# EXLYSHA/Recommendar-Systems

Hardware: AMD Instinct MI355X
Metric: BPR interactions/sec + full-sort items/sec, LightGCN d=64 at 1/2/4/8 MI355X (higher is better)
Workload: dtype f32; 1 GPU; C2: LightGCN K=3 d=64, sports-shaped (35,598 users x 18,357 items per rank), B=2048 per rank, device sampler, fused step; model=LightGCN, n_layers=3, embedding_size=64, global_batch=2048, per_rank_batch=2048, parallelism=single

## Files before the change

### recommendar-systems_amd/csrc/fullsort.hip

```cpp
#include <algorithm>
#include <climits>
#include <cstdlib>

#include "rsx_common.hpp"

namespace rsx {

typedef float floatx16 __attribute__((ext_vector_type(16)));
typedef unsigned long long u64;

constexpr int kCap = 256;
constexpr int kNK = kCap / 64;
constexpr int kSlack = 16;
constexpr int kWarm = 8;
constexpr int kMaxK = 96;

__device__ __forceinline__ unsigned ord_f32(float f) {
    const unsigned u = __float_as_uint(f);
    return (u & 0x80000000u) ? ~u : (u | 0x80000000u);
}
__device__ __forceinline__ float unord_f32(unsigned o) {
    const unsigned u = (o & 0x80000000u) ? (o & 0x7fffffffu) : ~o;
    return __uint_as_float(u);
}
// ... 12 lines not shown
    const unsigned lo = __shfl((unsigned)(v & 0xffffffffu), src, kWave);
    const unsigned hi = __shfl((unsigned)(v >> 32), src, kWave);
    return ((u64)hi << 32) | lo;
}

__device__ __forceinline__ void bitonic128_desc(u64& e0, u64& e1, int lane) {
#pragma unroll
    for (int size = 2; size <= 128; size <<= 1) {
#pragma unroll
        for (int stride = size >> 1; stride > 0; stride >>= 1) {
            if (stride == 64) {
                const u64 mx = e0 > e1 ? e0 : e1;
                const u64 mn = e0 > e1 ? e1 : e0;
                e0 = mx;
                e1 = mn;
            } else {
                const bool lower = (lane & stride) == 0;
                {
                    const u64 pv = shfl_xor_u64(e0, stride);
                    const bool desc = ((lane & size) == 0);
                    const bool keep_max = (lower == desc);
                    e0 = keep_max ? (e0 > pv ? e0 : pv) : (e0 > pv ? pv : e0);
                }
                {
                    const u64 pv = shfl_xor_u64(e1, stride);
                    const bool desc = (((lane + 64) & size) == 0);
                    const bool keep_max = (lower == desc);
                    e1 = keep_max ? (e1 > pv ? e1 : pv) : (e1 > pv ? pv : e1);
                }
            }
        }
    }
}

struct FsArgs {
    const float* U;
    const int64_t* users;
    int64_t nb;
    const float* I;
    int64_t ni;
    const int64_t* mrp;
    const int32_t* mcol;
    int k;
    int n_chunks;
    int64_t chunk_items;
    u64* cand;
    int* ccount;
    float* out_val;
    int64_t* out_idx;
    const __bf16* Ib;
    int n_lists;
    int seg_slots;
    int64_t seg_waves;
    unsigned* lbound;
    uint16_t* samp;
    uint16_t* mcnt1;
};


__device__ __forceinline__ int popc64(u64 x) { return __popcll(x); }
__device__ __forceinline__ u64 lanemask_lt(int lane) { return lane ? (~0ull >> (64 - lane)) : 0ull; }

__device__ __forceinline__ u64 ld_u64_l2(const u64* p) {
    return __hip_atomic_load(p, __ATOMIC_RELAXED, __HIP_MEMORY_SCOPE_AGENT);
}


__device__ __forceinline__ float compact_slot(u64* buf, int n, int k, int lane, int* new_cnt, unsigned lo,
                                              unsigned hi, int slack = -1) {
    asm volatile("s_waitcnt vmcnt(0)" ::: "memory");
    u64 x[kNK];
    unsigned hw[kNK];
#pragma unroll
    for (int q = 0; q < kNK; ++q) {
        x[q] = lane + 64 * q < n ? ld_u64_l2(buf + lane + 64 * q) : 0ull;
        hw[q] = (unsigned)(x[q] >> 32);
    }
    const unsigned diff = lo ^ hi;
    const int top = diff ? 31 - __builtin_clz(diff) : -1;
    unsigned th = top >= 31 ? 0u : (hi >> (top + 1)) << (top + 1);
    for (int bit = top; bit >= 0; --bit) {
        const unsigned c = th | (1u << bit);
        int m = 0;
#pragma unroll
        for (int q = 0; q < kNK; ++q) m += popc64(__ballot(hw[q] >= c));
        if (m >= k) {
            th = c;
            if (m <= k + slack) {
                const u64 lt = lanemask_lt(lane);
                int base = 0;
#pragma unroll
                for (int q = 0; q < kNK; ++q) {
                    const bool kp = x[q] != 0ull && hw[q] >= th;
                    const u64 bq = __ballot(kp);
                    if (kp) buf[base + popc64(bq & lt)] = x[q];
                    base += popc64(bq);
                }
                *new_cnt = base;
                return unord_f32(th);
            }
        }
    }
    int gt = 0, eq = 0;
#pragma unroll
    for (int q = 0; q < kNK; ++q) {
        gt += popc64(__ballot(hw[q] > th));
// ... 237 lines not shown
                    t2[r] = fmaxf(t2[r], lo);
                }
            }
            unsigned th = 0;
            for (int bit = 31; bit >= 0; --bit) {
                const unsigned c = th | (1u << bit);
                int n = 0;
#pragma unroll
                for (int r = 0; r < 16; ++r) n += (int)(ord_f32(t1[r]) >= c) + (int)(ord_f32(t2[r]) >= c);
                n += __shfl_xor(n, 32, kWave);
                if (n >= a.k) th = c;
            }
            if (uvalid && th > 0) {
                const float tb = unord_f32(th - 1);
                tau = tb == 0.f ? -__FLT_DENORM_MIN__ : tb;
            }
            mp = mp0;
            next_mask = nm0;
            load_chunk<D, CW>(ra, a.I, i0 + j, i1, a.ni, h * HALF, i0 + 32 <= i1);
        }
    }

    if (ntiles > 0) {
        floatx16 prev, cur;
        mfma_tile(IntC<0>{}, 0, prev);
        unsigned mb = mask_bits(i0);
        for (int t = 1; t < ntiles; ++t) {
            mfma_tile(IntC<0>{}, t, cur);
            filter(prev, mb, i0 + (int64_t)(t - 1) * 32);
            compact();
            mb = mask_bits(i0 + (int64_t)t * 32);
            prev = cur;
        }
        filter(prev, mb, i0 + (int64_t)(ntiles - 1) * 32);
        compact();
    }
    if (a.n_chunks > 2) {
        u64 need = __ballot(h == 0 && cnt > a.k);
        while (need) {
            const int jj = __ffsll((long long)need) - 1;
            need &= need - 1;
            const int n = __builtin_amdgcn_readlane(cnt, jj);
            const unsigned lo = (unsigned)__builtin_amdgcn_readlane((int)ord_f32(tau), jj);
            const unsigned hi = max((unsigned)__builtin_amdgcn_readlane((int)omax, jj),
                                    (unsigned)__builtin_amdgcn_readlane((int)omax, jj + 32));
            int kept;
            compact_slot(base + (int64_t)jj * rowstep, n, a.k, lane, &kept, lo, hi);
            if (j == jj) cnt = kept;
        }
    }
    if (uvalid && h == 0) a.ccount[bslot * a.n_chunks + chunk] = cnt;
}

constexpr int kScreenWpe = 2;
constexpr int kScreenTop = 3;
template <int D>
constexpr int kAbuf = D <= 64 ? 2 : 1;
typedef __bf16 bf16x8 __attribute__((ext_vector_type(8)));
typedef __bf16 bf16x2 __attribute__((ext_vector_type(2)));
typedef unsigned u32x4 __attribute__((ext_vector_type(4)));
constexpr float kScreenEps = 0.0080f;

template <int D>
constexpr int kScreenRow = D + 16;
constexpr int kScreenPadTiles = 2;

__device__ __forceinline__ unsigned pack_bf16x2(float lo, float hi) {
    const bf16x2 v = {(__bf16)lo, (__bf16)hi};
    return __builtin_bit_cast(unsigned, v);
}
__device__ __forceinline__ bf16x8 pack_bf16x8(float4 p, float4 q) {
    const u32x4 w = {pack_bf16x2(p.x, p.y), pack_bf16x2(p.z, p.w), pack_bf16x2(q.x, q.y), pack_bf16x2(q.z, q.w)};
    return __builtin_bit_cast(bf16x8, w);
}
__device__ __forceinline__ float vmax(float a, float b) {
    float r;
    asm("v_max_f32 %0, %1, %2" : "=v"(r) : "v"(a), "v"(b));
    return r;
}
__device__ __forceinline__ float vmed3(float a, float b, float c) {
    float r;
    asm("v_med3_f32 %0, %1, %2, %3" : "=v"(r) : "v"(a), "v"(b), "v"(c));
    return r;
}

__device__ __forceinline__ unsigned bf16_up(float x) { return (__float_as_uint(x) + 0xffffu) >> 16; }

template <int D>
__global__ __launch_bounds__(256) void fs_prep(const float* __restrict__ I, int64_t ni, int64_t ni_pad,
                                               __bf16* __restrict__ Ib) {
    constexpr int G = D / 4;
    constexpr int DP = kScreenRow<D>;
    const int64_t t = (int64_t)blockIdx.x * 256 + threadIdx.x;
    const int64_t row = t / G;
    const int c = (int)(t % G);
    const float4 v = row < ni ? ld4(I + row * D + 4 * c) : f4(0.f);
    float ss = v.x * v.x + v.y * v.y + v.z * v.z + v.w * v.w;
#pragma unroll
    for (int o = G / 2; o > 0; o >>= 1) ss += __shfl_xor(ss, o, kWave);
    if (row >= ni_pad) return;
    __bf16* r = Ib + row * DP;
    *reinterpret_cast<uint2*>(r + 4 * c) = make_uint2(pack_bf16x2(v.x, v.y), pack_bf16x2(v.z, v.w));
    if (c == 0) {
        const u32x4 z = {0u, 0u, 0u, 0u};
        u32x4 w = z;
        w[0] = bf16_up(sqrtf(ss) * 1.0001f);
        *reinterpret_cast<u32x4*>(r + D) = w;
        *reinterpret_cast<u32x4*>(r + D + 8) = z;
    }
}

template <int D, int ND>
__device__ __forceinline__ void exact_dots(const float* const (&u)[ND], const float* const (&v)[ND], float (&out)[ND]) {
    float acc[ND];
#pragma unroll
    for (int n = 0; n < ND; ++n) acc[n] = 0.f;
#pragma unroll 4
    for (int c = 0; c < D; c += 4) {
        float4 x[ND], y[ND];
#pragma unroll
        for (int n = 0; n < ND; ++n) {
            x[n] = *reinterpret_cast<const float4*>(u[n] + c);
            y[n] = ld4(v[n] + c);
        }
#pragma unroll
        for (int n = 0; n < ND; ++n) {
            acc[n] = fmaf(x[n].x, y[n].x, acc[n]);
            acc[n] = fmaf(x[n].y, y[n].y, acc[n]);
            acc[n] = fmaf(x[n].z, y[n].z, acc[n]);
            acc[n] = fmaf(x[n].w, y[n].w, acc[n]);
        }
    }
#pragma unroll
    for (int n = 0; n < ND; ++n) out[n] = acc[n];
}

constexpr int kDrainPer = 1;
constexpr int kQueueCap = 64 * kDrainPer + 1024;
constexpr int kMaskCap = 32;
constexpr int kMaskStride = kMaskCap + 1;

template <int D, int PH>
__device__ __forceinline__ void screen_segment(const FsArgs& a, int64_t ub, int chunk, int li, int ta, int tz,
                                               float* urows, unsigned* queue, int* lcnt, unsigned* lomax,
                                               int* mlds) {
    constexpr int HALF = D / 2;
    constexpr int NM = D / 16;
    constexpr int DP = kScreenRow<D>;
    constexpr int US = D + 4;
    const int lane = threadIdx.x, j = lane & 31, h = lane >> 5;
    const int64_t ublock = ub * 32;
    const int64_t bslot = ublock + j;
    const bool uvalid = bslot < a.nb;
    const int64_t urow = uvalid ? (a.users ? a.users[bslot] : bslot) : 0;
    const int64_t c0 = (int64_t)chunk * a.chunk_items;
    const int64_t i0 = c0 + (int64_t)ta * 32;
    const int64_t i1 = min(min(a.ni, c0 + a.chunk_items), c0 + (int64_t)tz * 32);
    const int ntiles = tz - ta;
    u64* const base = a.cand + (ublock * a.n_lists + li) * (int64_t)kCap;
    const int64_t rowstep = (int64_t)a.n_lists * kCap;

    u32x4 bu[NM + 1];
    float ss = 0.f;
    float* const myrow = urows + j * US;
#pragma unroll
    for (int s = 0; s < NM; ++s) {
        const float4 p = uvalid ? ld4(a.U + urow * D + h * HALF + 8 * s) : f4(0.f);
        const float4 q = uvalid ? ld4(a.U + urow * D + h * HALF + 8 * s + 4) : f4(0.f);
        ss += p.x * p.x + p.y * p.y + p.z * p.z + p.w * p.w + q.x * q.x + q.y * q.y + q.z * q.z + q.w * q.w;
        bu[s] = u32x4{pack_bf16x2(p.x, p.y), pack_bf16x2(p.z, p.w), pack_bf16x2(q.x, q.y), pack_bf16x2(q.z, q.w)};
        if constexpr (PH == 2) {
            *reinterpret_cast<float4*>(myrow + h * HALF + 8 * s) = p;
            *reinterpret_cast<float4*>(myrow + h * HALF + 8 * s + 4) = q;
        }
    }
    ss += __shfl_xor(ss, 32, kWave);
    const unsigned cmb = bf16_up(kScreenEps * sqrtf(ss) * 1.0001f);
    bu[NM] = u32x4{h == 0 ? (cmb | 0x8000u) : 0u, 0u, 0u, 0u};
    __syncthreads();

    int64_t mp = 0, me = 0, mq = 0;
    if (uvalid && a.mrp) {
        int64_t lo = a.mrp[urow], hi = a.mrp[urow + 1];
        me = hi;
        auto first_ge = [&](int64_t l, int64_t r, int64_t x) __attribute__((always_inline)) {
            while (l < r) {
                const int64_t mid = (l + r) >> 1;
                if ((int64_t)a.mcol[mid] < x) l = mid + 1; else r = mid;
            }
            return l;
        };
        mp = first_ge(lo, hi, i0);
        mq = first_ge(mp, hi, i1);
    }
    const int64_t mcount = mq - mp;
    const int kk = a.k + (int)mcount;
    const bool mfree = __ballot(uvalid && kk > 32 * kScreenTop) == 0ull;
    const bool mlds_ok = __ballot(mcount > kMaskCap) == 0ull;
    int* const ml = mlds + j * kMaskStride;
    if (mlds_ok) {
        int v[kMaskCap / 2];
        if (mcount > 0) {
#pragma unroll
            for (int q = 0; q < kMaskCap / 2; ++q) v[q] = a.mcol[mp + min((int64_t)(2 * q + h), mcount - 1)];
        }
#pragma unroll
        for (int q = 0; q < kMaskCap / 2; ++q) ml[2 * q + h] = 2 * q + h < mcount ? v[q] : INT_MAX;
        if (h == 0) ml[kMaskCap] = INT_MAX;
    }
    const int64_t mp0 = mp;
    int next_mask = INT_MAX, after = INT_MAX, mcur = 0;
    auto mask_start = [&]() __attribute__((always_inline)) {
        const int nm = mlds_ok ? ml[0] : (mp0 < me ? a.mcol[mp0] : INT_MAX);
        const int af = (!mlds_ok && mp0 + 1 < me) ? a.mcol[mp0 + 1] : INT_MAX;
        mcur = 0;
        mp = mp0;
        next_mask = nm;
        after = af;
    };
    __syncthreads();
    mask_start();
    auto mask_bits = [&](auto form, int64_t tb) __attribute__((always_inline)) -> unsigned {
        constexpr int M = decltype(form)::value;
        unsigned mb = 0;
        if constexpr (M == 1) {
            while ((int64_t)next_mask < tb + 32) {
                mb |= 1u << (unsigned)((int64_t)next_mask - tb);
                next_mask = ml[++mcur];
            }
        } else if constexpr (M == 2) {
            while ((int64_t)next_mask < tb + 32) {
                mb |= 1u << (unsigned)((int64_t)next_mask - tb);
                ++mp;
                next_mask = after;
                after = mp + 1 < me ? a.mcol[mp + 1] : INT_MAX;
            }
        }
        return mb;
    };
    constexpr int NB = kAbuf<D>;
    static_assert(NB == 1 || NB == 2, "the ring below is written for one or two buffers");
    u32x4 ra[NB][NM + 1];
    const __bf16* const a0 = a.Ib + (i0 + j) * DP;
    const __bf16* anext = a0;
    auto load_a = [&](auto par) __attribute__((always_inline)) {
        constexpr int P = decltype(par)::value % NB;
        const u32x4* p = reinterpret_cast<const u32x4*>(anext + h * HALF);
#pragma unroll
        for (int s = 0; s < NM; ++s) ra[P][s] = p[s];
        ra[P][NM] = *reinterpret_cast<const u32x4*>(anext + D + 8 * h);
        anext += 32 * DP;
    };
    auto tile = [&](auto par, int t, floatx16& acc) __attribute__((always_inline)) {
        constexpr int P = decltype(par)::value % NB;
        if constexpr (NB > 1) load_a(IntC<(P + NB - 1) % NB>{});
#pragma unroll
        for (int r = 0; r < 16; ++r) acc[r] = 0.f;
#pragma unroll
        for (int s = 0; s <= NM; ++s)
            acc = __builtin_amdgcn_mfma_f32_32x32x16_bf16(__builtin_bit_cast(bf16x8, ra[P][s]),
                                                          __builtin_bit_cast(bf16x8, bu[s]), acc, 0, 0, 0);
        if constexpr (NB == 1) load_a(IntC<0>{});
    };
    auto prime = [&]() __attribute__((always_inline)) {
        anext = a0;
        if (ntiles <= 0) return;
        load_a(IntC<0>{});
    };
    auto sweep = [&](auto&& body) __attribute__((always_inline)) {
        for (int t = 0; t < ntiles; t += NB) {
            body(IntC<0>{}, t);
            if constexpr (NB > 1)
                if (t + 1 < ntiles) body(IntC<1>{}, t + 1);
        }
    };

    float t1[16], t2[16], t3[16];
#pragma unroll
    for (int r = 0; r < 16; ++r) t1[r] = t2[r] = t3[r] = -INFINITY;
    auto p1_issue = [&](auto form, auto par, int t, floatx16& acc) __attribute__((always_inline)) -> unsigned {
        const unsigned mb = mask_bits(form, i0 + (int64_t)t * 32);
        tile(par, t, acc);
        return mb;
    };
    auto p1_update = [&](auto form, int t, floatx16& acc, unsigned mb) __attribute__((always_inline)) {
        const int64_t tb = i0 + (int64_t)t * 32;
        const int rem = (int)(i1 - tb);
        if (rem < 32 || (decltype(form)::value != 0 && __ballot(mb != 0u) != 0ull)) {
            const unsigned mbh = mb >> (4 * h);
            const int remh = rem - 4 * h;
#pragma unroll
            for (int r = 0; r < 16; ++r) {
                const int io = (r & 3) + 8 * (r >> 2);
                acc[r] = io >= remh ? -INFINITY : (((mbh >> io) & 1u) ? -1e10f : acc[r]);
            }
        }
#pragma unroll
        for (int r = 0; r < 16; ++r) {
            t3[r] = vmed3(t2[r], t3[r], acc[r]);
            t2[r] = vmed3(t1[r], t2[r], acc[r]);
            t1[r] = vmax(t1[r], acc[r]);
        }
    };
    auto pass1 = [&](auto form, auto par, int t) __attribute__((always_inline)) {
        floatx16 acc;
        const unsigned mb = p1_issue(form, par, t, acc);
        p1_update(form, t, acc, mb);
    };
    auto sweep1 = [&](auto form) __attribute__((always_inline)) {
        sweep([&](auto par, int t) __attribute__((always_inline)) { pass1(form, par, t); });
    };
    if constexpr (PH == 1) {
        prime();
        if (mfree) sweep1(IntC<0>{});
        else if (mlds_ok) sweep1(IntC<1>{});
        else sweep1(IntC<2>{});
        if (uvalid) {
            auto s16 = [](float x) __attribute__((always_inline)) -> unsigned {
                return x == -INFINITY ? 0u : ord_f32(x) >> 16;
            };
            uint4* dst = reinterpret_cast<uint4*>(a.samp + ((bslot * a.n_lists + li) * 96 + h * 48));
#pragma unroll
            for (int q = 0; q < 6; ++q) {
                unsigned w[4];
#pragma unroll
                for (int e = 0; e < 4; ++e) {
                    const int v0 = 8 * q + 2 * e, v1 = v0 + 1;
                    const float x0 = v0 < 16 ? t1[v0] : v0 < 32 ? t2[v0 - 16] : t3[v0 - 32];
                    const float x1 = v1 < 16 ? t1[v1] : v1 < 32 ? t2[v1 - 16] : t3[v1 - 32];
                    w[e] = s16(x0) | (s16(x1) << 16);
                }
                dst[q] = make_uint4(w[0], w[1], w[2], w[3]);
            }
            if (h == 0) a.mcnt1[bslot * a.n_lists + li] = (uint16_t)(mfree ? min(mcount, (int64_t)0xfffe) : 0);
        }
        return;
    }
    const unsigned th = uvalid ? a.lbound[bslot] : 0u;
    float tau = -INFINITY;
    if (th > ord_f32(-INFINITY)) {
        const float tb = unord_f32(th - 1);
        tau = tb == 0.f ? -__FLT_DENORM_MIN__ : tb;
    }

    bu[NM] = u32x4{h == 0 ? cmb : 0u, 0u, 0u, 0u};
    mask_start();
    int cnt = 0;
    unsigned omax = 0;
    if (lane < 32) {
        lcnt[lane] = 0;
        lomax[lane] = 0u;
    }
    int qn = 0;
    auto compact = [&]() __attribute__((always_inline)) {
        u64 need = __ballot(h == 0 && cnt > kCap - 64 * kDrainPer);
        while (need) {
            const int jj = __ffsll((long long)need) - 1;
            need &= need - 1;
            const int nn = __builtin_amdgcn_readlane(cnt, jj);
            const unsigned lo = (unsigned)__builtin_amdgcn_readlane((int)ord_f32(tau), jj);
            const unsigned hi = (unsigned)__builtin_amdgcn_readlane((int)omax, jj);
            int kept;
            const float nt = compact_slot(base + (int64_t)jj * rowstep, nn, a.k, lane, &kept, lo, hi, kSlack);
            if (j == jj) {
                tau = nt;
                cnt = kept;
            }
            if (lane == jj) lcnt[jj] = kept;
        }
    };
    const u64 ltm = lanemask_lt(lane);
    auto drain = [&](bool all) __attribute__((always_inline)) {
        constexpr int G = 64 * kDrainPer;
        int g = 0;
        while (qn - g >= G || (all && qn > g)) {
            const int n = min(G, qn - g);
            __syncthreads();
            unsigned e[kDrainPer];
            int ju[kDrainPer];
            float tj[kDrainPer], sc[kDrainPer];
            const float* up[kDrainPer];
            const float* vp[kDrainPer];
#pragma unroll
            for (int q = 0; q < kDrainPer; ++q) {
                e[q] = lane + 64 * q < n ? queue[g + lane + 64 * q] : 0u;
                ju[q] = (int)(e[q] & 31u);
                tj[q] = __shfl(tau, ju[q], kWave);
                up[q] = urows + ju[q] * US;
                vp[q] = a.I + (int64_t)(e[q] >> 6) * D;
            }
            if (lane < n) {
                exact_dots<D, kDrainPer>(up, vp, sc);
            }
#pragma unroll
            for (int q = 0; q < kDrainPer; ++q) {
                const float v = (e[q] & 32u) ? -1e10f : sc[q];
                if (lane + 64 * q < n && v > tj[q]) {
                    const int pos = atomicAdd(&lcnt[ju[q]], 1);
                    const u64 key = make_key(v, (int)(e[q] >> 6));
                    atomicMax(&lomax[ju[q]], (unsigned)(key >> 32));
                    base[(int64_t)ju[q] * rowstep + pos] = key;
                }
            }
            __syncthreads();
            cnt = lcnt[j];
            omax = lomax[j];
            compact();
            g += n;
        }
        const int rest = qn - g;
        if (g > 0 && rest > 0) {
            unsigned v[kDrainPer];
            __syncthreads();
#pragma unroll
            for (int q = 0; q < kDrainPer; ++q) v[q] = lane + 64 * q < rest ? queue[g + lane + 64 * q] : 0u;
            __syncthreads();
#pragma unroll
            for (int q = 0; q < kDrainPer; ++q)
                if (lane + 64 * q < rest) queue[lane + 64 * q] = v[q];
        }
        qn = rest;
    };
    auto pass2 = [&](auto form, auto par, int t) __attribute__((always_inline)) {
        const int64_t tb = i0 + (int64_t)t * 32;
        const unsigned mb = mask_bits(form, tb);
        floatx16 acc;
        tile(par, t, acc);
        const int rem = (int)(i1 - tb);
        const unsigned ebase = ((unsigned)(tb + 4 * h) << 6) | (unsigned)j;
        auto push = [&](bool c, unsigned e) __attribute__((always_inline)) {
            const u64 bal = __ballot(c);
            if (bal) {
                const int rk = __builtin_amdgcn_mbcnt_hi((unsigned)(bal >> 32), __builtin_amdgcn_mbcnt_lo((unsigned)bal, 0u));
                if (c) queue[qn + rk] = e;
                qn += popc64(bal);
            }
        };
        const float tv = uvalid ? tau : INFINITY;
        const unsigned mbh = mb >> (4 * h);
        if (rem < 32 || __ballot(tv < -1e10f) != 0ull) {
            const int remh = rem - 4 * h;
#pragma unroll
            for (int r = 0; r < 16; ++r) {
                const int io = (r & 3) + 8 * (r >> 2);
                acc[r] = io >= remh ? -INFINITY : (((mbh >> io) & 1u) ? -1e10f : acc[r]);
            }
        }
#pragma unroll
        for (int r = 0; r < 16; ++r) {
            const int io = (r & 3) + 8 * (r >> 2);
            push(acc[r] > tv, (ebase + ((unsigned)io << 6)) | (((mbh >> io) & 1u) << 5));
        }
        if (qn >= 64 * kDrainPer) drain(false);
    };
    prime();
    if (mlds_ok) sweep([&](auto par, int t) __attribute__((always_inline)) { pass2(IntC<1>{}, par, t); });
    else sweep([&](auto par, int t) __attribute__((always_inline)) { pass2(IntC<2>{}, par, t); });
    drain(true);
    __syncthreads();
    cnt = lcnt[j];
    omax = lomax[j];
    if (a.n_lists > 8) {
        u64 need = __ballot(h == 0 && cnt > a.k);
        while (need) {
            const int jj = __ffsll((long long)need) - 1;
            need &= need - 1;
            const int nn = __builtin_amdgcn_readlane(cnt, jj);
            const unsigned lo = (unsigned)__builtin_amdgcn_readlane((int)ord_f32(tau), jj);
            const unsigned hi = max((unsigned)__builtin_amdgcn_readlane((int)omax, jj),
                                    (unsigned)__builtin_amdgcn_readlane((int)omax, jj + 32));
            int kept;
            compact_slot(base + (int64_t)jj * rowstep, nn, a.k, lane, &kept, lo, hi);
            if (j == jj) cnt = kept;
        }
    }
    if (uvalid && h == 0) a.ccount[bslot * a.n_lists + li] = cnt;
    __syncthreads();
}

template <int D, int PH>
__global__ __launch_bounds__(64) __attribute__((amdgpu_waves_per_eu(D <= 64 ? kScreenWpe : 1))) void fs_screen(FsArgs a) {
    constexpr int US = D + 4;
    __shared__ __attribute__((aligned(16))) float urows[PH == 1 ? 4 : 32 * US];
    __shared__ unsigned queue[PH == 1 ? 1 : kQueueCap];
    __shared__ int lcnt[32];
    __shared__ unsigned lomax[32];
    __shared__ int mlds[32 * kMaskStride];
    const int64_t n_ub = (a.nb + 31) / 32;
    const int64_t nper = a.seg_waves ? a.seg_waves : n_ub;
    int64_t w;
    int chunk;
    if ((8 % a.n_chunks) == 0) {
        const int64_t b = blockIdx.x, xcd = b & 7, slot = b >> 3;
        chunk = (int)(xcd % a.n_chunks);
        w = slot * (8 / a.n_chunks) + xcd / a.n_chunks;
    } else {
        chunk = (int)(blockIdx.x % a.n_chunks);
        w = blockIdx.x / a.n_chunks;
    }
    if (w >= nper) return;
    const int64_t c0 = (int64_t)chunk * a.chunk_items;
    const int nt = (int)((min(a.ni, c0 + a.chunk_items) - c0 + 31) / 32);
    const int64_t T = n_ub * nt;
    const int64_t lo = a.seg_waves ? w * T / nper : w * nt, hi = a.seg_waves ? (w + 1) * T / nper : (w + 1) * nt;
    const int S = a.seg_slots;
    for (int64_t x = lo; x < hi;) {
        const int64_t ub = x / nt;
        const int t0 = (int)(x - ub * nt);
        const int t1 = (int)min((int64_t)nt, t0 + (hi - x));
        const int64_t wf = ((ub * nt + 1) * nper + T - 1) / T - 1;
        const int seg = a.seg_waves ? (int)(w - wf) : 0;
        screen_segment<D, PH>(a, ub, chunk, chunk * S + seg, t0, t1, urows, queue, lcnt, lomax, mlds);
        if (PH == 2 && t1 == nt) {
            const int j = threadIdx.x & 31;
            const int64_t bslot = ub * 32 + j;
            if (threadIdx.x < 32 && bslot < a.nb)
                for (int q = seg + 1; q < S; ++q) a.ccount[bslot * a.n_lists + chunk * S + q] = 0;
        }
        x += t1 - t0;
    }
}

template <int NW>
__global__ __launch_bounds__(256) void fs_thresh(const uint16_t* __restrict__ samp, const uint16_t* __restrict__ mcnt,
                                                 int nl, int64_t nb, int k, unsigned* __restrict__ lbound) {
    const int lane = threadIdx.x & 63;
    const int64_t b = (int64_t)blockIdx.x * 4 + (threadIdx.x >> 6);
    if (b >= nb) return;
    const unsigned m = lane < nl ? (unsigned)mcnt[b * nl + lane] : 0xffffu;
    const u64 valid = __ballot(m != 0xffffu);
    int mm = m != 0xffffu ? (int)m : 0;
#pragma unroll
    for (int o = 32; o > 0; o >>= 1) mm += __shfl_xor(mm, o, kWave);
    const int kk = k + mm;
    const int nwords = nl * 48;
    const unsigned* __restrict__ w32 = reinterpret_cast<const unsigned*>(samp) + b * nwords;
    unsigned v[2 * NW];
#pragma unroll
    for (int q = 0; q < NW; ++q) {
        const int e = lane + 64 * q;
        const unsigned x = e < nwords ? w32[e] : 0u;
        const bool ok = e < nwords && ((valid >> (e / 48)) & 1ull);
        v[2 * q] = ok ? (x & 0xffffu) : 0u;
        v[2 * q + 1] = ok ? (x >> 16) : 0u;
    }
    unsigned th = 0;
    for (int bit = 15; bit >= 0; --bit) {
        const unsigned c = th | (1u << bit);
        int n = 0;
#pragma unroll
        for (int q = 0; q < 2 * NW; ++q) n += popc64(__ballot(v[q] >= c));
        if (n >= kk) th = c;
    }
    if (lane == 0) lbound[b] = th << 16;
}

template <int E>
__device__ __forceinline__ u64 kth_largest_n(const u64 (&e)[E], int k) {
    unsigned hi = 0u, lo = 0xffffffffu;
#pragma unroll
    for (int m = 0; m < E; ++m) {
        const unsigned w = (unsigned)(e[m] >> 32);
        if (e[m] != 0ull) {
            hi = max(hi, w);
            lo = min(lo, w);
        }
    }
#pragma unroll
    for (int o = kWave / 2; o > 0; o >>= 1) {
// ... 129 lines not shown
            base += popc64(bal);
        }
    } else {
        for (int p0 = 0; p0 < total; p0 += 64) {
            const u64 x = p0 + lane < total ? Ls.at(p0 + lane) : 0ull;
            const bool kp = x != 0ull && x >= T;
            const u64 bal = __ballot(kp);
            if (kp) top[wv][base + popc64(bal & lt)] = x;
            base += popc64(bal);
        }
    }
    __builtin_amdgcn_wave_barrier();
    __builtin_amdgcn_fence(__ATOMIC_SEQ_CST, "wavefront");
    const int kept = base;
    for (int q = lane; q < kept; q += 64) {
        const u64 mine = top[wv][q];
        int r = 0;
        for (int t = 0; t < kept; ++t) r += top[wv][t] > mine;
        a.out_val[b * k + r] = key_score(mine);
        a.out_idx[b * k + r] = (int64_t)key_index(mine);
    }
    for (int q = kept + lane; q < k; q += 64) {
        a.out_val[b * k + q] = -INFINITY;
        a.out_idx[b * k + q] = -1;
    }
}

static void fs_plan(int64_t nb, int64_t ni, int d, int* n_chunks, int64_t* chunk_items) {
    const int64_t waves = (nb + 31) / 32;
    const int64_t target = d <= 64 ? 1900 : 950;
    int64_t s = (target + waves - 1) / waves;
    if (s < 1) s = 1;
    if (s > 16) s = 16;
    int64_t per = (ni + s - 1) / s;
    per = (per + 31) / 32 * 32;
    if (per < 32) per = 32;
    *chunk_items = per;
    *n_chunks = (int)((ni + per - 1) / per);
}

static bool fs_use_screen(int k, int d, int64_t ni) {
    return k <= 64 && (d == 32 || d == 64 || d == 128 || d == 256) && ni < (1ll << 26);
}

static size_t fs_align(size_t x) { return (x + 255) / 256 * 256; }

struct FsLayout {
    int n_chunks;
    int64_t chunk_items;
    bool screen;
    int n_lists, seg_slots;
    int64_t seg_waves;
    int64_t blocks;
};

static int fs_cus() {
    static int n = 0;
    if (!n) {
        int dev = 0, v = 0;
        n = (hipGetDevice(&dev) == hipSuccess &&
             hipDeviceGetAttribute(&v, hipDeviceAttributeMultiprocessorCount, dev) == hipSuccess && v > 0)
                ? v
                : 256;
        (void)hipGetLastError();
    }
    return n;
}

static void screen_plan(int64_t nb, int64_t ni, int wps, int* n_chunks, int64_t* chunk_items) {
    const int64_t n_ub = (nb + 31) / 32;
    const int64_t slots = (int64_t)fs_cus() * 4 * wps;
    int64_t c = slots / n_ub;
    if (c < 1 || n_ub * c * 5 < slots * 4) c = (slots + n_ub - 1) / n_ub;
    if (c < 1) c = 1;
    if (c > 16) c = 16;
    int64_t per = (ni + c - 1) / c;
    per = (per + 31) / 32 * 32;
    *chunk_items = per;
    *n_chunks = (int)((ni + per - 1) / per);
}

static int fs_wps(int d) { return d <= 128 ? 2 : 1; }

static FsLayout fs_layout(int64_t nb, int64_t ni, int k, int d) {
    FsLayout L{};
    const int wps = fs_wps(d);
    L.screen = fs_use_screen(k, d, ni);
    if (L.screen) screen_plan(nb, ni, wps, &L.n_chunks, &L.chunk_items);
    else fs_plan(nb, ni, d, &L.n_chunks, &L.chunk_items);
    L.n_lists = L.n_chunks;
    L.seg_slots = 1;
    const int64_t n_ub = (nb + 31) / 32;
    const int C = L.n_chunks;
    L.blocks = n_ub * C;
    if (L.screen && (8 % C) == 0) {
        const int64_t slots = (int64_t)fs_cus() * 4 * wps;
        const int64_t wc = slots / C;
        if (n_ub * C > slots && wc >= 1) {
            int S = 1;
            bool ok = true;
            for (int c = 0; c < C; ++c) {
                const int64_t nt = (std::min(ni, (int64_t)(c + 1) * L.chunk_items) - (int64_t)c * L.chunk_items + 31) / 32;
                const int64_t m = n_ub * nt / wc;
                if (m < 1) ok = false;
                else S = (int)std::max<int64_t>(S, (nt + m - 1) / m + 1);
            }
            if (ok && C * S <= 8) {
                L.seg_waves = wc;
                L.seg_slots = S;
                L.n_lists = C * S;
                L.blocks = wc * C;
            }
        }
    }
    if ((8 % C) == 0) L.blocks = (L.blocks + 7) / 8 * 8;
    return L;
}

size_t fs_ws(int64_t nb, int64_t ni, int k, int d) {
    const FsLayout L = fs_layout(nb, ni, k, d);
    const int nl = L.n_lists;
    size_t bytes = fs_align((size_t)nb * nl * kCap * sizeof(u64) + (size_t)nb * nl * sizeof(int) + 512);
    if (L.screen) {
        const size_t ni_pad = (size_t)(ni + 31) / 32 * 32;
        bytes += fs_align((ni_pad + 32 * kScreenPadTiles) * (d + 16) * sizeof(__bf16));
        bytes += fs_align((size_t)nb * sizeof(unsigned));
        bytes += fs_align((size_t)nb * L.n_lists * 96 * sizeof(uint16_t));
        bytes += fs_align((size_t)nb * L.n_lists * sizeof(uint16_t));
    }
    return bytes;
}

template <int D>
static int launch_fs(const FsArgs& a, const FsLayout& L, hipStream_t s) {
    const dim3 grid((unsigned)L.blocks);
    if (a.Ib) {
        const int64_t ni_pad = (a.ni + 31) / 32 * 32;
        const int64_t nthr = ni_pad * (D / 4);
        hipLaunchKernelGGL((fs_prep<D>), dim3((unsigned)((nthr + 255) / 256)), dim3(256), 0, s, a.I, a.ni, ni_pad,
                           const_cast<__bf16*>(a.Ib));
        (void)hipMemsetAsync(a.mcnt1, 0xff, (size_t)a.nb * L.n_lists * sizeof(uint16_t), s);
        hipLaunchKernelGGL((fs_screen<D, 1>), grid, dim3(64), 0, s, a);
        {
            const dim3 tg((unsigned)((a.nb + 3) / 4));
            const uint16_t* sp = a.samp;
            const uint16_t* mc = a.mcnt1;
            const int nl = L.n_lists;
            if (nl <= 4) hipLaunchKernelGGL((fs_thresh<3>), tg, dim3(256), 0, s, sp, mc, nl, a.nb, a.k, a.lbound);
            else if (nl <= 8) hipLaunchKernelGGL((fs_thresh<6>), tg, dim3(256), 0, s, sp, mc, nl, a.nb, a.k, a.lbound);
            else hipLaunchKernelGGL((fs_thresh<12>), tg, dim3(256), 0, s, sp, mc, nl, a.nb, a.k, a.lbound);
        }
        hipLaunchKernelGGL((fs_screen<D, 2>), grid, dim3(64), 0, s, a);
    } else {
        hipLaunchKernelGGL((fs_tiles<D>), grid, dim3(64), 0, s, a);
    }
    const dim3 sg((unsigned)((a.nb + 3) / 4));
    const int n = a.n_lists;
    if (n <= 2) hipLaunchKernelGGL((fs_select<2>), sg, dim3(256), 0, s, a);
    else if (n <= 4) hipLaunchKernelGGL((fs_select<4>), sg, dim3(256), 0, s, a);
    else if (n <= 8) hipLaunchKernelGGL((fs_select<8>), sg, dim3(256), 0, s, a);
    else hipLaunchKernelGGL((fs_select<16>), sg, dim3(256), 0, s, a);
    return last_rc();
}

int fs_call(const float* U, const int64_t* users, int64_t nb, const float* I, int64_t ni, int d,
            const int64_t* mrp, const int32_t* mcol, int k, float* out_val, int64_t* out_idx, void* ws,
            size_t ws_bytes, hipStream_t s) {
    if (!U || !I || !out_val || !out_idx || nb < 0 || ni <= 0 || k <= 0) return RSX_ERR_ARG;
    if (k > ni) return RSX_ERR_ARG;
    if (k > kMaxK) return RSX_ERR_UNSUPPORTED;
    if (nb == 0) return RSX_OK;
    if (!ws || ws_bytes < fs_ws(nb, ni, k, d)) return RSX_ERR_WORKSPACE;
    FsArgs a;
    const FsLayout L = fs_layout(nb, ni, k, d);
    const int nl = L.n_lists;
    a.n_chunks = L.n_chunks;
    a.chunk_items = L.chunk_items;
    a.n_lists = L.n_lists;
    a.seg_slots = L.seg_slots;
    a.seg_waves = L.seg_waves;
    a.U = U;
    a.users = users;
    a.nb = nb;
    a.I = I;
    a.ni = ni;
    a.mrp = mrp;
    a.mcol = mcol;
    a.k = k;
    a.cand = static_cast<u64*>(ws);
    a.ccount = reinterpret_cast<int*>(static_cast<char*>(ws) + (size_t)nb * nl * kCap * sizeof(u64));
    a.out_val = out_val;
    a.out_idx = out_idx;
    a.Ib = nullptr;
    a.lbound = nullptr;
    a.samp = nullptr;
    a.mcnt1 = nullptr;
    if (L.screen) {
        char* p = static_cast<char*>(ws) + fs_align((size_t)nb * nl * kCap * sizeof(u64) + (size_t)nb * nl * sizeof(int) + 512);
        a.Ib = reinterpret_cast<const __bf16*>(p);
        const size_t ni_pad = (size_t)(ni + 31) / 32 * 32;
        char* q = p + fs_align((ni_pad + 32 * kScreenPadTiles) * (d + 16) * sizeof(__bf16));
        a.lbound = reinterpret_cast<unsigned*>(q);
        q += fs_align((size_t)nb * sizeof(unsigned));
        a.samp = reinterpret_cast<uint16_t*>(q);
        q += fs_align((size_t)nb * L.n_lists * 96 * sizeof(uint16_t));
        a.mcnt1 = reinterpret_cast<uint16_t*>(q);
    }
    switch (d) {
        case 32: return launch_fs<32>(a, L, s);
        case 64: return launch_fs<64>(a, L, s);
        case 128: return launch_fs<128>(a, L, s);
        case 256: return launch_fs<256>(a, L, s);
        default: return RSX_ERR_UNSUPPORTED;
    }
}

template <int D>
__global__ __launch_bounds__(256) void score_dense(const float* __restrict__ U, const int64_t* __restrict__ users,
                                                   int64_t nb, const float* __restrict__ I, int64_t ni,
                                                   float* __restrict__ out) {
    __shared__ float urow[D];
    const int64_t b = blockIdx.y;
    const int64_t ur = users ? users[b] : b;
    for (int c = threadIdx.x; c < D; c += 256) urow[c] = U[ur * D + c];
    __syncthreads();
    const int64_t i = (int64_t)blockIdx.x * 256 + threadIdx.x;
    if (i >= ni) return;
    const float* ir = I + i * D;
    float acc = 0.f;
#pragma unroll 8
    for (int c = 0; c < D; c += 4) {
        const float4 v = ld4(ir + c);
        acc = fmaf(urow[c], v.x, acc);
        acc = fmaf(urow[c + 1], v.y, acc);
        acc = fmaf(urow[c + 2], v.z, acc);
        acc = fmaf(urow[c + 3], v.w, acc);
    }
    out[b * ni + i] = acc;
}

__global__ void gather_rows_k(const float* __restrict__ src, const int64_t* __restrict__ idx, int64_t n,
                              int64_t offset, int d, float* __restrict__ out) {
    const int64_t t = (int64_t)blockIdx.x * blockDim.x + threadIdx.x;
    const int64_t r = t / d;
    if (r >= n) return;
    const int c = (int)(t % d);
    out[r * d + c] = src[(idx[r] + offset) * d + c];
}

}

extern "C" {

size_t rsx_fullsort_ws_bytes(int64_t n_batch, int64_t n_items, int32_t k) {
    size_t w = 0;
    for (int d : {32, 64, 128, 256}) {
        const size_t b = rsx::fs_ws(n_batch, n_items, k, d);
        w = b > w ? b : w;
// ... 47 lines not shown
```

Baseline: 15.40 million interactions/s.

## Process two user blocks per wave in screen pass one with separate segment plan

```diff
diff --git a/recommendar-systems_amd/csrc/fullsort.hip b/recommendar-systems_amd/csrc/fullsort.hip
--- a/recommendar-systems_amd/csrc/fullsort.hip
+++ b/recommendar-systems_amd/csrc/fullsort.hip
@@ -88,6 +88,8 @@
     int n_lists;
     int seg_slots;
     int64_t seg_waves;
+    int n_lists1, seg_slots1;
+    int64_t seg_waves1;
     unsigned* lbound;
     uint16_t* samp;
     uint16_t* mcnt1;
@@ -431,7 +433,6 @@
     if (uvalid && h == 0) a.ccount[bslot * a.n_chunks + chunk] = cnt;
 }
 
-constexpr int kScreenWpe = 2;
 constexpr int kScreenTop = 3;
 template <int D>
 constexpr int kAbuf = D <= 64 ? 2 : 1;
@@ -518,20 +519,28 @@
 constexpr int kQueueCap = 64 * kDrainPer + 1024;
 constexpr int kMaskCap = 32;
 constexpr int kMaskStride = kMaskCap + 1;
-
-template <int D, int PH>
-__device__ __forceinline__ void screen_segment(const FsArgs& a, int64_t ub, int chunk, int li, int ta, int tz,
+template <int D>
+constexpr int kScreenUB = D <= 64 ? 2 : 1;
+
+template <int D, int PH, int UB>
+__device__ __forceinline__ void screen_segment(const FsArgs& a, int64_t unit, int chunk, int li, int ta, int tz,
                                                float* urows, unsigned* queue, int* lcnt, unsigned* lomax,
                                                int* mlds) {
     constexpr int HALF = D / 2;
     constexpr int NM = D / 16;
     constexpr int DP = kScreenRow<D>;
     constexpr int US = D + 4;
+    constexpr int NU = 32 * UB;
     const int lane = threadIdx.x, j = lane & 31, h = lane >> 5;
-    const int64_t ublock = ub * 32;
-    const int64_t bslot = ublock + j;
-    const bool uvalid = bslot < a.nb;
-    const int64_t urow = uvalid ? (a.users ? a.users[bslot] : bslot) : 0;
+    const int64_t ublock = unit * NU;
+    int64_t bslots[UB], urow[UB];
+    bool uvalids[UB];
+#pragma unroll
+    for (int b = 0; b < UB; ++b) {
+        bslots[b] = ublock + 32 * b + j;
+        uvalids[b] = bslots[b] < a.nb;
+        urow[b] = uvalids[b] ? (a.users ? a.users[bslots[b]] : bslots[b]) : 0;
+    }
     const int64_t c0 = (int64_t)chunk * a.chunk_items;
     const int64_t i0 = c0 + (int64_t)ta * 32;
     const int64_t i1 = min(min(a.ni, c0 + a.chunk_items), c0 + (int64_t)tz * 32);
@@ -539,80 +548,102 @@
     u64* const base = a.cand + (ublock * a.n_lists + li) * (int64_t)kCap;
     const int64_t rowstep = (int64_t)a.n_lists * kCap;
 
-    u32x4 bu[NM + 1];
-    float ss = 0.f;
-    float* const myrow = urows + j * US;
-#pragma unroll
-    for (int s = 0; s < NM; ++s) {
-        const float4 p = uvalid ? ld4(a.U + urow * D + h * HALF + 8 * s) : f4(0.f);
-        const float4 q = uvalid ? ld4(a.U + urow * D + h * HALF + 8 * s + 4) : f4(0.f);
-        ss += p.x * p.x + p.y * p.y + p.z * p.z + p.w * p.w + q.x * q.x + q.y * q.y + q.z * q.z + q.w * q.w;
-        bu[s] = u32x4{pack_bf16x2(p.x, p.y), pack_bf16x2(p.z, p.w), pack_bf16x2(q.x, q.y), pack_bf16x2(q.z, q.w)};
-        if constexpr (PH == 2) {
-            *reinterpret_cast<float4*>(myrow + h * HALF + 8 * s) = p;
-            *reinterpret_cast<float4*>(myrow + h * HALF + 8 * s + 4) = q;
-        }
-    }
-    ss += __shfl_xor(ss, 32, kWave);
-    const unsigned cmb = bf16_up(kScreenEps * sqrtf(ss) * 1.0001f);
-    bu[NM] = u32x4{h == 0 ? (cmb | 0x8000u) : 0u, 0u, 0u, 0u};
+    u32x4 bus[UB][NM + 1];
+    unsigned cmbs[UB];
+#pragma unroll
+    for (int b = 0; b < UB; ++b) {
+        float ss = 0.f;
+        float* const myrow = urows + (32 * b + j) * US;
+#pragma unroll
+        for (int s = 0; s < NM; ++s) {
+            const float4 p = uvalids[b] ? ld4(a.U + urow[b] * D + h * HALF + 8 * s) : f4(0.f);
+            const float4 q = uvalids[b] ? ld4(a.U + urow[b] * D + h * HALF + 8 * s + 4) : f4(0.f);
+            ss += p.x * p.x + p.y * p.y + p.z * p.z + p.w * p.w + q.x * q.x + q.y * q.y + q.z * q.z + q.w * q.w;
+            bus[b][s] = u32x4{pack_bf16x2(p.x, p.y), pack_bf16x2(p.z, p.w), pack_bf16x2(q.x, q.y), pack_bf16x2(q.z, q.w)};
+            if constexpr (PH == 2) {
+                *reinterpret_cast<float4*>(myrow + h * HALF + 8 * s) = p;
+                *reinterpret_cast<float4*>(myrow + h * HALF + 8 * s + 4) = q;
+            }
+        }
+        ss += __shfl_xor(ss, 32, kWave);
+        cmbs[b] = bf16_up(kScreenEps * sqrtf(ss) * 1.0001f);
+        bus[b][NM] = u32x4{h == 0 ? (cmbs[b] | 0x8000u) : 0u, 0u, 0u, 0u};
+    }
     __syncthreads();
 
-    int64_t mp = 0, me = 0, mq = 0;
-    if (uvalid && a.mrp) {
-        int64_t lo = a.mrp[urow], hi = a.mrp[urow + 1];
-        me = hi;
-        auto first_ge = [&](int64_t l, int64_t r, int64_t x) __attribute__((always_inline)) {
-            while (l < r) {
-                const int64_t mid = (l + r) >> 1;
-                if ((int64_t)a.mcol[mid] < x) l = mid + 1; else r = mid;
-            }
-            return l;
-        };
-        mp = first_ge(lo, hi, i0);
-        mq = first_ge(mp, hi, i1);
-    }
-    const int64_t mcount = mq - mp;
-    const int kk = a.k + (int)mcount;
-    const bool mfree = __ballot(uvalid && kk > 32 * kScreenTop) == 0ull;
-    const bool mlds_ok = __ballot(mcount > kMaskCap) == 0ull;
-    int* const ml = mlds + j * kMaskStride;
-    if (mlds_ok) {
-        int v[kMaskCap / 2];
-        if (mcount > 0) {
-#pragma unroll
-            for (int q = 0; q < kMaskCap / 2; ++q) v[q] = a.mcol[mp + min((int64_t)(2 * q + h), mcount - 1)];
-        }
-#pragma unroll
-        for (int q = 0; q < kMaskCap / 2; ++q) ml[2 * q + h] = 2 * q + h < mcount ? v[q] : INT_MAX;
-        if (h == 0) ml[kMaskCap] = INT_MAX;
-    }
-    const int64_t mp0 = mp;
-    int next_mask = INT_MAX, after = INT_MAX, mcur = 0;
+    int64_t mp[UB], me[UB], mcount[UB];
+    bool over_top = false, over_cap = false;
+#pragma unroll
+    for (int b = 0; b < UB; ++b) {
+        int64_t mq = 0;
+        mp[b] = me[b] = 0;
+        if (uvalids[b] && a.mrp) {
+            int64_t lo = a.mrp[urow[b]], hi = a.mrp[urow[b] + 1];
+            me[b] = hi;
+            auto first_ge = [&](int64_t l, int64_t r, int64_t x) __attribute__((always_inline)) {
+                while (l < r) {
+                    const int64_t mid = (l + r) >> 1;
+                    if ((int64_t)a.mcol[mid] < x) l = mid + 1; else r = mid;
+                }
+                return l;
+            };
+            mp[b] = first_ge(lo, hi, i0);
+            mq = first_ge(mp[b], hi, i1);
+        }
+        mcount[b] = mq - mp[b];
+        over_top |= uvalids[b] && a.k + (int)mcount[b] > 32 * kScreenTop;
+        over_cap |= mcount[b] > kMaskCap;
+    }
+    const bool mfree = __ballot(over_top) == 0ull;
+    const bool mlds_ok = __ballot(over_cap) == 0ull;
+    int* ml[UB];
+#pragma unroll
+    for (int b = 0; b < UB; ++b) {
+        ml[b] = mlds + (32 * b + j) * kMaskStride;
+        if (mlds_ok) {
+            int v[kMaskCap / 2];
+            if (mcount[b] > 0) {
+#pragma unroll
+                for (int q = 0; q < kMaskCap / 2; ++q)
+                    v[q] = a.mcol[mp[b] + min((int64_t)(2 * q + h), mcount[b] - 1)];
+            }
+#pragma unroll
+            for (int q = 0; q < kMaskCap / 2; ++q) ml[b][2 * q + h] = 2 * q + h < mcount[b] ? v[q] : INT_MAX;
+            if (h == 0) ml[b][kMaskCap] = INT_MAX;
+        }
+    }
+    int64_t mp0[UB];
+    int next_mask[UB], after[UB], mcur[UB];
+#pragma unroll
+    for (int b = 0; b < UB; ++b) mp0[b] = mp[b];
     auto mask_start = [&]() __attribute__((always_inline)) {
-        const int nm = mlds_ok ? ml[0] : (mp0 < me ? a.mcol[mp0] : INT_MAX);
-        const int af = (!mlds_ok && mp0 + 1 < me) ? a.mcol[mp0 + 1] : INT_MAX;
-        mcur = 0;
-        mp = mp0;
-        next_mask = nm;
-        after = af;
+#pragma unroll
+        for (int b = 0; b < UB; ++b) {
+            const int nm = mlds_ok ? ml[b][0] : (mp0[b] < me[b] ? a.mcol[mp0[b]] : INT_MAX);
+            const int af = (!mlds_ok && mp0[b] + 1 < me[b]) ? a.mcol[mp0[b] + 1] : INT_MAX;
+            mcur[b] = 0;
+            mp[b] = mp0[b];
+            next_mask[b] = nm;
+            after[b] = af;
+        }
     };
     __syncthreads();
     mask_start();
-    auto mask_bits = [&](auto form, int64_t tb) __attribute__((always_inline)) -> unsigned {
+    auto mask_bits = [&](auto form, auto blk, int64_t tb) __attribute__((always_inline)) -> unsigned {
         constexpr int M = decltype(form)::value;
+        constexpr int B = decltype(blk)::value;
         unsigned mb = 0;
         if constexpr (M == 1) {
-            while ((int64_t)next_mask < tb + 32) {
-                mb |= 1u << (unsigned)((int64_t)next_mask - tb);
-                next_mask = ml[++mcur];
+            while ((int64_t)next_mask[B] < tb + 32) {
+                mb |= 1u << (unsigned)((int64_t)next_mask[B] - tb);
+                next_mask[B] = ml[B][++mcur[B]];
             }
         } else if constexpr (M == 2) {
-            while ((int64_t)next_mask < tb + 32) {
-                mb |= 1u << (unsigned)((int64_t)next_mask - tb);
-                ++mp;
-                next_mask = after;
-                after = mp + 1 < me ? a.mcol[mp + 1] : INT_MAX;
+            while ((int64_t)next_mask[B] < tb + 32) {
+                mb |= 1u << (unsigned)((int64_t)next_mask[B] - tb);
+                ++mp[B];
+                next_mask[B] = after[B];
+                after[B] = mp[B] + 1 < me[B] ? a.mcol[mp[B] + 1] : INT_MAX;
             }
         }
         return mb;
@@ -630,15 +661,24 @@
         ra[P][NM] = *reinterpret_cast<const u32x4*>(anext + D + 8 * h);
         anext += 32 * DP;
     };
-    auto tile = [&](auto par, int t, floatx16& acc) __attribute__((always_inline)) {
+    auto mfmas = [&](auto par, auto blk, floatx16& acc) __attribute__((always_inline)) {
+        constexpr int P = decltype(par)::value % NB;
+        constexpr int B = decltype(blk)::value;
+#pragma unroll
+        for (int r = 0; r < 16; ++r) acc[r] = 0.f;
+#pragma unroll
+        for (int s = 0; s <= NM; ++s)
+            acc = __builtin_amdgcn_mfma_f32_32x32x16_bf16(__builtin_bit_cast(bf16x8, ra[P][s]),
+                                                          __builtin_bit_cast(bf16x8, bus[B][s]), acc, 0, 0, 0);
+    };
+    auto tile = [&](auto par, floatx16* acc, auto&& between) __attribute__((always_inline)) {
         constexpr int P = decltype(par)::value % NB;
         if constexpr (NB > 1) load_a(IntC<(P + NB - 1) % NB>{});
-#pragma unroll
-        for (int r = 0; r < 16; ++r) acc[r] = 0.f;
-#pragma unroll
-        for (int s = 0; s <= NM; ++s)
-            acc = __builtin_amdgcn_mfma_f32_32x32x16_bf16(__builtin_bit_cast(bf16x8, ra[P][s]),
-                                                          __builtin_bit_cast(bf16x8, bu[s]), acc, 0, 0, 0);
+        mfmas(par, IntC<0>{}, acc[0]);
+        if constexpr (UB == 2) {
+            between();
+            mfmas(par, IntC<1>{}, acc[1]);
+        }
         if constexpr (NB == 1) load_a(IntC<0>{});
     };
     auto prime = [&]() __attribute__((always_inline)) {
@@ -654,15 +694,13 @@
         }
     };
 
-    float t1[16], t2[16], t3[16];
-#pragma unroll
-    for (int r = 0; r < 16; ++r) t1[r] = t2[r] = t3[r] = -INFINITY;
-    auto p1_issue = [&](auto form, auto par, int t, floatx16& acc) __attribute__((always_inline)) -> unsigned {
-        const unsigned mb = mask_bits(form, i0 + (int64_t)t * 32);
-        tile(par, t, acc);
-        return mb;
-    };
-    auto p1_update = [&](auto form, int t, floatx16& acc, unsigned mb) __attribute__((always_inline)) {
+    float t1[UB][16], t2[UB][16], t3[UB][16];
+#pragma unroll
+    for (int b = 0; b < UB; ++b)
+#pragma unroll
+        for (int r = 0; r < 16; ++r) t1[b][r] = t2[b][r] = t3[b][r] = -INFINITY;
+    auto p1_update = [&](auto form, auto blk, int t, floatx16& acc, unsigned mb) __attribute__((always_inline)) {
+        constexpr int B = decltype(blk)::value;
         const int64_t tb = i0 + (int64_t)t * 32;
         const int rem = (int)(i1 - tb);
         if (rem < 32 || (decltype(form)::value != 0 && __ballot(mb != 0u) != 0ull)) {
@@ -676,45 +714,67 @@
         }
 #pragma unroll
         for (int r = 0; r < 16; ++r) {
-            t3[r] = vmed3(t2[r], t3[r], acc[r]);
-            t2[r] = vmed3(t1[r], t2[r], acc[r]);
-            t1[r] = vmax(t1[r], acc[r]);
-        }
-    };
+            t3[B][r] = vmed3(t2[B][r], t3[B][r], acc[r]);
+            t2[B][r] = vmed3(t1[B][r], t2[B][r], acc[r]);
+            t1[B][r] = vmax(t1[B][r], acc[r]);
+        }
+    };
+    floatx16 acc1[UB];
+    unsigned mbp = 0;
+    int tp = -1;
     auto pass1 = [&](auto form, auto par, int t) __attribute__((always_inline)) {
-        floatx16 acc;
-        const unsigned mb = p1_issue(form, par, t, acc);
-        p1_update(form, t, acc, mb);
+        unsigned mb[UB];
+        mb[0] = mask_bits(form, IntC<0>{}, i0 + (int64_t)t * 32);
+        if constexpr (UB == 2) mb[1] = mask_bits(form, IntC<1>{}, i0 + (int64_t)t * 32);
+        tile(par, acc1, [&]() __attribute__((always_inline)) { p1_update(form, IntC<UB - 1>{}, tp, acc1[UB - 1], mbp); });
+        p1_update(form, IntC<0>{}, t, acc1[0], mb[0]);
+        if constexpr (UB == 2) {
+            mbp = mb[1];
+            tp = t;
+        }
     };
     auto sweep1 = [&](auto form) __attribute__((always_inline)) {
+        if constexpr (UB == 2) {
+#pragma unroll
+            for (int r = 0; r < 16; ++r) acc1[1][r] = -INFINITY;
+        }
         sweep([&](auto par, int t) __attribute__((always_inline)) { pass1(form, par, t); });
+        if constexpr (UB == 2) p1_update(form, IntC<UB - 1>{}, tp, acc1[UB - 1], mbp);
     };
     if constexpr (PH == 1) {
         prime();
         if (mfree) sweep1(IntC<0>{});
         else if (mlds_ok) sweep1(IntC<1>{});
         else sweep1(IntC<2>{});
-        if (uvalid) {
+#pragma unroll
+        for (int b = 0; b < UB; ++b) {
+            if (!uvalids[b]) continue;
             auto s16 = [](float x) __attribute__((always_inline)) -> unsigned {
                 return x == -INFINITY ? 0u : ord_f32(x) >> 16;
             };
-            uint4* dst = reinterpret_cast<uint4*>(a.samp + ((bslot * a.n_lists + li) * 96 + h * 48));
+            uint4* dst = reinterpret_cast<uint4*>(a.samp + ((bslots[b] * a.n_lists1 + li) * 96 + h * 48));
 #pragma unroll
             for (int q = 0; q < 6; ++q) {
                 unsigned w[4];
 #pragma unroll
                 for (int e = 0; e < 4; ++e) {
                     const int v0 = 8 * q + 2 * e, v1 = v0 + 1;
-                    const float x0 = v0 < 16 ? t1[v0] : v0 < 32 ? t2[v0 - 16] : t3[v0 - 32];
-                    const float x1 = v1 < 16 ? t1[v1] : v1 < 32 ? t2[v1 - 16] : t3[v1 - 32];
+                    const float x0 = v0 < 16 ? t1[b][v0] : v0 < 32 ? t2[b][v0 - 16] : t3[b][v0 - 32];
+                    const float x1 = v1 < 16 ? t1[b][v1] : v1 < 32 ? t2[b][v1 - 16] : t3[b][v1 - 32];
                     w[e] = s16(x0) | (s16(x1) << 16);
                 }
                 dst[q] = make_uint4(w[0], w[1], w[2], w[3]);
             }
-            if (h == 0) a.mcnt1[bslot * a.n_lists + li] = (uint16_t)(mfree ? min(mcount, (int64_t)0xfffe) : 0);
+            if (h == 0)
+                a.mcnt1[bslots[b] * a.n_lists1 + li] = (uint16_t)(mfree ? min(mcount[b], (int64_t)0xfffe) : 0);
         }
         return;
     }
+    static_assert(PH == 1 || UB == 1, "pass 2 is written for one user block a wave");
+    const bool uvalid = uvalids[0];
+    const int64_t bslot = bslots[0];
+    const unsigned cmb = cmbs[0];
+    u32x4(&bu)[NM + 1] = bus[0];
     const unsigned th = uvalid ? a.lbound[bslot] : 0u;
     float tau = -INFINITY;
     if (th > ord_f32(-INFINITY)) {
@@ -802,9 +862,9 @@
     };
     auto pass2 = [&](auto form, auto par, int t) __attribute__((always_inline)) {
         const int64_t tb = i0 + (int64_t)t * 32;
-        const unsigned mb = mask_bits(form, tb);
+        const unsigned mb = mask_bits(form, IntC<0>{}, tb);
         floatx16 acc;
-        tile(par, t, acc);
+        tile(par, &acc, [] {});
         const int rem = (int)(i1 - tb);
         const unsigned ebase = ((unsigned)(tb + 4 * h) << 6) | (unsigned)j;
         auto push = [&](bool c, unsigned e) __attribute__((always_inline)) {
@@ -858,15 +918,19 @@
 }
 
 template <int D, int PH>
-__global__ __launch_bounds__(64) __attribute__((amdgpu_waves_per_eu(D <= 64 ? kScreenWpe : 1))) void fs_screen(FsArgs a) {
+__global__ __launch_bounds__(64) __attribute__((amdgpu_waves_per_eu(PH == 2 && D <= 64 ? 2 : 1))) void fs_screen(FsArgs a) {
     constexpr int US = D + 4;
-    __shared__ __attribute__((aligned(16))) float urows[PH == 1 ? 4 : 32 * US];
+    constexpr int UB = PH == 1 ? kScreenUB<D> : 1;
+    constexpr int NU = 32 * UB;
+    const int64_t seg_waves = PH == 1 ? a.seg_waves1 : a.seg_waves;
+    const int S = PH == 1 ? a.seg_slots1 : a.seg_slots;
+    __shared__ __attribute__((aligned(16))) float urows[PH == 1 ? 4 : NU * US];
     __shared__ unsigned queue[PH == 1 ? 1 : kQueueCap];
-    __shared__ int lcnt[32];
-    __shared__ unsigned lomax[32];
-    __shared__ int mlds[32 * kMaskStride];
-    const int64_t n_ub = (a.nb + 31) / 32;
-    const int64_t nper = a.seg_waves ? a.seg_waves : n_ub;
+    __shared__ int lcnt[NU];
+    __shared__ unsigned lomax[NU];
+    __shared__ int mlds[NU * kMaskStride];
+    const int64_t n_un = (a.nb + NU - 1) / NU;
+    const int64_t nper = seg_waves ? seg_waves : n_un;
     int64_t w;
     int chunk;
     if ((8 % a.n_chunks) == 0) {
@@ -880,20 +944,18 @@
     if (w >= nper) return;
     const int64_t c0 = (int64_t)chunk * a.chunk_items;
     const int nt = (int)((min(a.ni, c0 + a.chunk_items) - c0 + 31) / 32);
-    const int64_t T = n_ub * nt;
-    const int64_t lo = a.seg_waves ? w * T / nper : w * nt, hi = a.seg_waves ? (w + 1) * T / nper : (w + 1) * nt;
-    const int S = a.seg_slots;
+    const int64_t T = n_un * nt;
+    const int64_t lo = seg_waves ? w * T / nper : w * nt, hi = seg_waves ? (w + 1) * T / nper : (w + 1) * nt;
     for (int64_t x = lo; x < hi;) {
-        const int64_t ub = x / nt;
-        const int t0 = (int)(x - ub * nt);
+        const int64_t un = x / nt;
+        const int t0 = (int)(x - un * nt);
         const int t1 = (int)min((int64_t)nt, t0 + (hi - x));
-        const int64_t wf = ((ub * nt + 1) * nper + T - 1) / T - 1;
-        const int seg = a.seg_waves ? (int)(w - wf) : 0;
-        screen_segment<D, PH>(a, ub, chunk, chunk * S + seg, t0, t1, urows, queue, lcnt, lomax, mlds);
+        const int64_t wf = ((un * nt + 1) * nper + T - 1) / T - 1;
+        const int seg = seg_waves ? (int)(w - wf) : 0;
+        screen_segment<D, PH, UB>(a, un, chunk, chunk * S + seg, t0, t1, urows, queue, lcnt, lomax, mlds);
         if (PH == 2 && t1 == nt) {
-            const int j = threadIdx.x & 31;
-            const int64_t bslot = ub * 32 + j;
-            if (threadIdx.x < 32 && bslot < a.nb)
+            const int64_t bslot = un * NU + threadIdx.x;
+            if (threadIdx.x < NU && bslot < a.nb)
                 for (int q = seg + 1; q < S; ++q) a.ccount[bslot * a.n_lists + chunk * S + q] = 0;
         }
         x += t1 - t0;
@@ -1129,6 +1191,8 @@
     int n_lists, seg_slots;
     int64_t seg_waves;
     int64_t blocks;
+    int n_lists1, seg_slots1;
+    int64_t seg_waves1, blocks1;
 };
 
 static int fs_cus() {
@@ -1144,6 +1208,7 @@
     return n;
 }
 
+static int fs_plan_wps(int d) { return d <= 128 ? 2 : 1; }
 static void screen_plan(int64_t nb, int64_t ni, int wps, int* n_chunks, int64_t* chunk_items) {
     const int64_t n_ub = (nb + 31) / 32;
     const int64_t slots = (int64_t)fs_cus() * 4 * wps;
@@ -1157,40 +1222,54 @@
     *n_chunks = (int)((ni + per - 1) / per);
 }
 
-static int fs_wps(int d) { return d <= 128 ? 2 : 1; }
+static int fs_ub1(int d) { return d <= 64 ? 2 : 1; }
+static int fs_wps1(int d) { return d <= 64 ? 1 : fs_plan_wps(d); }
+
+static int64_t fs_split(int64_t n_un, int C, int64_t ni, int64_t chunk_items, int64_t slots, int64_t* seg_waves,
+                        int* seg_slots) {
+    *seg_waves = 0;
+    *seg_slots = 1;
+    int64_t blocks = n_un * C;
+    const int64_t wc = slots / C;
+    if ((8 % C) == 0 && n_un * C > slots && wc >= 1) {
+        int S = 1;
+        bool ok = true;
+        for (int c = 0; c < C; ++c) {
+            const int64_t nt = (std::min(ni, (int64_t)(c + 1) * chunk_items) - (int64_t)c * chunk_items + 31) / 32;
+            const int64_t m = n_un * nt / wc;
+            if (m < 1) ok = false;
+            else S = (int)std::max<int64_t>(S, (nt + m - 1) / m + 1);
+        }
+        if (ok && C * S <= 8) {
+            *seg_waves = wc;
+            *seg_slots = S;
+            blocks = wc * C;
+        }
+    }
+    if ((8 % C) == 0) blocks = (blocks + 7) / 8 * 8;
+    return blocks;
+}
 
 static FsLayout fs_layout(int64_t nb, int64_t ni, int k, int d) {
     FsLayout L{};
-    const int wps = fs_wps(d);
     L.screen = fs_use_screen(k, d, ni);
-    if (L.screen) screen_plan(nb, ni, wps, &L.n_chunks, &L.chunk_items);
+    if (L.screen) screen_plan(nb, ni, fs_plan_wps(d), &L.n_chunks, &L.chunk_items);
     else fs_plan(nb, ni, d, &L.n_chunks, &L.chunk_items);
-    L.n_lists = L.n_chunks;
-    L.seg_slots = 1;
     const int64_t n_ub = (nb + 31) / 32;
     const int C = L.n_chunks;
-    L.blocks = n_ub * C;
-    if (L.screen && (8 % C) == 0) {
-        const int64_t slots = (int64_t)fs_cus() * 4 * wps;
-        const int64_t wc = slots / C;
-        if (n_ub * C > slots && wc >= 1) {
-            int S = 1;
-            bool ok = true;
-            for (int c = 0; c < C; ++c) {
-                const int64_t nt = (std::min(ni, (int64_t)(c + 1) * L.chunk_items) - (int64_t)c * L.chunk_items + 31) / 32;
-                const int64_t m = n_ub * nt / wc;
-                if (m < 1) ok = false;
-                else S = (int)std::max<int64_t>(S, (nt + m - 1) / m + 1);
-            }
-            if (ok && C * S <= 8) {
-                L.seg_waves = wc;
-                L.seg_slots = S;
-                L.n_lists = C * S;
-                L.blocks = wc * C;
-            }
-        }
-    }
-    if ((8 % C) == 0) L.blocks = (L.blocks + 7) / 8 * 8;
+    L.n_lists = L.n_lists1 = C;
+    L.seg_slots = L.seg_slots1 = 1;
+    L.blocks = L.blocks1 = n_ub * C;
+    if (L.screen) {
+        L.blocks = fs_split(n_ub, C, ni, L.chunk_items, (int64_t)fs_cus() * 4 * fs_plan_wps(d), &L.seg_waves, &L.seg_slots);
+        L.n_lists = C * L.seg_slots;
+        const int ub = fs_ub1(d);
+        L.blocks1 = fs_split((n_ub + ub - 1) / ub, C, ni, L.chunk_items, (int64_t)fs_cus() * 4 * fs_wps1(d),
+                             &L.seg_waves1, &L.seg_slots1);
+        L.n_lists1 = C * L.seg_slots1;
+    } else if ((8 % C) == 0) {
+        L.blocks = (L.blocks + 7) / 8 * 8;
+    }
     return L;
 }
 
@@ -1202,8 +1281,8 @@
         const size_t ni_pad = (size_t)(ni + 31) / 32 * 32;
         bytes += fs_align((ni_pad + 32 * kScreenPadTiles) * (d + 16) * sizeof(__bf16));
         bytes += fs_align((size_t)nb * sizeof(unsigned));
-        bytes += fs_align((size_t)nb * L.n_lists * 96 * sizeof(uint16_t));
-        bytes += fs_align((size_t)nb * L.n_lists * sizeof(uint16_t));
+        bytes += fs_align((size_t)nb * L.n_lists1 * 96 * sizeof(uint16_t));
+        bytes += fs_align((size_t)nb * L.n_lists1 * sizeof(uint16_t));
     }
     return bytes;
 }
@@ -1216,13 +1295,13 @@
         const int64_t nthr = ni_pad * (D / 4);
         hipLaunchKernelGGL((fs_prep<D>), dim3((unsigned)((nthr + 255) / 256)), dim3(256), 0, s, a.I, a.ni, ni_pad,
                            const_cast<__bf16*>(a.Ib));
-        (void)hipMemsetAsync(a.mcnt1, 0xff, (size_t)a.nb * L.n_lists * sizeof(uint16_t), s);
-        hipLaunchKernelGGL((fs_screen<D, 1>), grid, dim3(64), 0, s, a);
+        (void)hipMemsetAsync(a.mcnt1, 0xff, (size_t)a.nb * L.n_lists1 * sizeof(uint16_t), s);
+        hipLaunchKernelGGL((fs_screen<D, 1>), dim3((unsigned)L.blocks1), dim3(64), 0, s, a);
         {
             const dim3 tg((unsigned)((a.nb + 3) / 4));
             const uint16_t* sp = a.samp;
             const uint16_t* mc = a.mcnt1;
-            const int nl = L.n_lists;
+            const int nl = L.n_lists1;
             if (nl <= 4) hipLaunchKernelGGL((fs_thresh<3>), tg, dim3(256), 0, s, sp, mc, nl, a.nb, a.k, a.lbound);
             else if (nl <= 8) hipLaunchKernelGGL((fs_thresh<6>), tg, dim3(256), 0, s, sp, mc, nl, a.nb, a.k, a.lbound);
             else hipLaunchKernelGGL((fs_thresh<12>), tg, dim3(256), 0, s, sp, mc, nl, a.nb, a.k, a.lbound);
@@ -1256,6 +1335,9 @@
     a.n_lists = L.n_lists;
     a.seg_slots = L.seg_slots;
     a.seg_waves = L.seg_waves;
+    a.n_lists1 = L.n_lists1;
+    a.seg_slots1 = L.seg_slots1;
+    a.seg_waves1 = L.seg_waves1;
     a.U = U;
     a.users = users;
     a.nb = nb;
@@ -1280,7 +1362,7 @@
         a.lbound = reinterpret_cast<unsigned*>(q);
         q += fs_align((size_t)nb * sizeof(unsigned));
         a.samp = reinterpret_cast<uint16_t*>(q);
-        q += fs_align((size_t)nb * L.n_lists * 96 * sizeof(uint16_t));
+        q += fs_align((size_t)nb * L.n_lists1 * 96 * sizeof(uint16_t));
         a.mcnt1 = reinterpret_cast<uint16_t*>(q);
     }
     switch (d) {
```

Measured after the change: 15.40 million interactions/s (median of 4 runs). About the same (+0.0%).
